# SchusterLab/quantum-optimal-control

Measured on AMD Instinct MI355X. Metric: GRAPE iterations/sec (fwd+bwd+Adam) at n=32 k=4 steps=500, higher is better.
Workload: dtype f64; 1 GPU; C2 3-transmon-size unitary gate: n=32 k=4 steps=500 m=8 Taylor(T,s)=(5,3), 64 independent control seeds per GPU (aggregate over seeds), reg_coeffs={}; seeds_per_gpu=64, total_seeds=64, chunks=16, stream_groups=1, ranks_seen=1, fidelities_gathered=64, devices_distinct=1, transport=single process, transport_fallback=False

## Files before the change

quantum-optimal-control_amd/csrc/qoc_engine.hip:

```cpp
#include "../../include/qoc.h"

#include <hip/hip_runtime.h>

#include <cmath>
#include <cstdarg>
#include <cstdio>
#include <cstdlib>
#include <cstring>
#include <string>
#include <vector>

#include "qoc_common.h"
#include "qoc_kernels_finish.h"
#include "qoc_kernels_generic.h"
#include "qoc_kernels_mfma.h"
#include "qoc_kernels_st.h"
#include "qoc_kernels_gemm.h"
#include "qoc_gemm_ts.h"
#include "qoc_small.h"

#include "qoc_plan_limits.h"
static thread_local std::string g_err;

static int fail(int code, const char* fmt, ...) {
// ... 182 lines not shown
    }
    if (d.has_speed) {
        const size_t g = ((size_t)d.B * (d.steps + 1) + 3) / 4;
        hipLaunchKernelGGL(k_time_overlaps, dim3((unsigned)(g > 4096 ? 4096 : g)), dim3(256), 0, s, d);
    }
    hipLaunchKernelGGL(k_loss, dim3(d.B), dim3(QOC_BLOCK), 0, s, d);
}

static int enqueue_small(qoc_engine* e, const QocAdamDev& ap, int iters) {
    QocDev d = e->d;
    d.skip_done = ap.mode == 1 ? 1 : 0;
    std::string msg;
    TRY(prof_begin(e));
    const int rc = qoc_small_launch(e->sm, d, ap, iters, e->stream, msg);
    if (rc) return fail(rc == -1 ? QOC_ERR_INVALID : QOC_ERR_HIP, "workgroup-resident iteration: %s", msg.c_str());
    TRY(prof_end(e));
    HIP_TRY(hipGetLastError());
    e->evaluated = true;
    e->controls_ready = false;
    e->final_stale = true;
    e->inter_stale = true;
    return QOC_OK;
}

static int enqueue_iteration(qoc_engine* e, const QocAdamDev& ap) {
    if (e->path == QOC_PATH_SMALL) return enqueue_small(e, ap, 1);
    const bool own_controls = e->path == QOC_PATH_MFMA && e->mf.latency && e->mf.NT == 2;
    const bool swap_in = e->controls_ready && !own_controls && !(e->skip_mask & 1);
    if (swap_in) { std::swap(e->d.u, e->d.u2); std::swap(e->d.w, e->d.w2); }
    e->controls_ready = false;
    QocDev d = e->d;
    if (own_controls) { d.u2 = nullptr; d.w2 = nullptr; }
    d.skip_done = ap.mode == 1 ? 1 : 0;
    d.uscale_in_loss = (e->path == QOC_PATH_MFMA && !e->mf.latency && !e->mf.updown) ? 1 : 0;
    const int total = d.B * d.k * d.steps;
    int cgrid = (total + QOC_BLOCK - 1) / QOC_BLOCK;
    if (cgrid > 2048) cgrid = 2048;
    const int skip = e->skip_mask;
    const bool plain = !(d.has_amp || d.has_env || d.has_dwdt || d.has_d2wdt2 || d.has_band);
    const bool fused_tail = e->path == QOC_PATH_MFMA && e->mf.latency && (!e->mf.lat_sources || e->mf.lat_src_fast) && !d.has_band
        && !(skip & (16 | 32));
    if (!(skip & 1) && !own_controls && !swap_in) hipLaunchKernelGGL(k_controls, dim3(cgrid), dim3(QOC_BLOCK), 0, e->stream, d);
    if (e->path == QOC_PATH_MFMA) {
        TRY(prof_begin(e));
        if (!(skip & 2)) qoc_mfma_launch_expm(e->mf, d, e->stream);
        TRY(prof_end(e));
// ... 22 lines not shown
        qoc_gemm_backward(e->gm, d, e->stream);
        if (bracket_bwd) TRY(prof_end(e));
        }
    } else if (!d.state_transfer) {
        TRY(prof_begin(e));
        hipLaunchKernelGGL(k_expm_generic, dim3(e->expm_grid), dim3(QOC_BLOCK), 0, e->stream, d, e->K, e->expm_scratch);
        TRY(prof_end(e));
        hipLaunchKernelGGL(k_fwd_generic, dim3(d.B), dim3(QOC_BLOCK), 0, e->stream, d, e->K, e->seed_scratch);
        launch_loss(d, e->stream);
        hipLaunchKernelGGL(k_bwd_generic, dim3(d.B), dim3(QOC_BLOCK), 0, e->stream, d, e->K, e->seed_scratch);
    } else if (e->path == QOC_PATH_ST_FUSED) {
        TRY(prof_begin(e));
        st_fused_launch(d, e->stream, true);
        TRY(prof_end(e));
        launch_loss(d, e->stream);
        st_fused_launch(d, e->stream, false);
    } else {
        TRY(prof_begin(e));
        hipLaunchKernelGGL(k_st_fwd_generic, dim3(d.B), dim3(QOC_BLOCK), 0, e->stream, d, e->seed_scratch);
        TRY(prof_end(e));
        launch_loss(d, e->stream);
        hipLaunchKernelGGL(k_st_bwd_generic, dim3(d.B), dim3(QOC_BLOCK), 0, e->stream, d, e->seed_scratch);
    }
    if (!(skip & 32) && !fused_tail) {
        const dim3 fb(d.k * d.steps >= 2048 ? 1024 : QOC_BLOCK);
        if (d.has_band) {
            const size_t items = (size_t)d.B * d.k * d.steps, g1 = (items + 3) / 4, g2 = (items + 255) / 256;
            hipLaunchKernelGGL(k_band_spectrum, dim3((unsigned)(g1 > 8192 ? 8192 : g1)), dim3(256), 0, e->stream, d);
            hipLaunchKernelGGL(k_band_gradient, dim3((unsigned)(g2 > 8192 ? 8192 : g2)), dim3(256), 0, e->stream, d);
        }
        const bool wide = d.k * d.steps > 4 * 1024 && d.k * d.steps <= 8 * 1024;
        const bool split = d.k * d.steps > 4 * 1024 && e->fin_part;
        if (split) {
            const dim3 sg((unsigned)e->fin_S, (unsigned)d.B);
            QocGradPartial gp{nullptr, 0, 0, 0};
            if (e->path == QOC_PATH_GEMM && e->gm.reduce_in_tail) gp = QocGradPartial{e->gm.partial, e->gm.N / 32, e->gm.ldW, e->gm.MV};
            if (plain) {
                hipLaunchKernelGGL(k_finish_split_a<true>, sg, dim3(256), 0, e->stream, d, ap, e->fin_part, gp);
                hipLaunchKernelGGL(k_finish_split_b<true>, sg, dim3(256), 0, e->stream, d, ap, e->fin_part);
            } else {
                hipLaunchKernelGGL(k_finish_split_a<false>, sg, dim3(256), 0, e->stream, d, ap, e->fin_part, gp);
                hipLaunchKernelGGL(k_finish_split_b<false>, sg, dim3(256), 0, e->stream, d, ap, e->fin_part);
            }
        }
        else if (plain && wide) hipLaunchKernelGGL((k_finish_t<true, 8>), dim3(d.B), fb, 0, e->stream, d, ap);
        else if (plain) hipLaunchKernelGGL(k_finish_t<true>, dim3(d.B), fb, 0, e->stream, d, ap);
        else if (wide) hipLaunchKernelGGL((k_finish_t<false, 8>), dim3(d.B), fb, 0, e->stream, d, ap);
        else hipLaunchKernelGGL(k_finish_t<false>, dim3(d.B), fb, 0, e->stream, d, ap);
    }
    HIP_TRY(hipGetLastError());
    e->evaluated = true;
    e->controls_ready = ap.mode != 0 && !own_controls && !(skip & (16 | 32));
    e->final_stale = (e->path == QOC_PATH_MFMA && (e->mf.latency || e->mf.updown)) ||
                     (e->path == QOC_PATH_GEMM && e->gm.ts_G <= 0 && qoc_gemm_lazy_final(e->gm, e->d));
    e->inter_stale = (e->path == QOC_PATH_MFMA && e->final_stale && (!e->mf.lat_sources || e->mf.lat_src_fast))
// ... 161 lines not shown
        ident.assign(2 * nn, 0.0);
        for (int a = 0; a < n; ++a) ident[2 * (a * n + a)] = 1.0;
        U0 = ident.data();
    }
    if ((rc = dev_upload(e, &d.Hs, (const cplx*)Hs, (size_t)(k + 1) * nn))) return bail(rc);
    if ((rc = dev_upload(e, &d.U0, (const cplx*)U0, nn))) return bail(rc);
    if ((rc = dev_upload(e, &d.V, (const cplx*)V, nm))) return bail(rc);
    if ((rc = dev_upload(e, &d.W, (const cplx*)W, nm))) return bail(rc);
    if ((rc = dev_upload(e, &d.Psi0, (const cplx*)psi0.data(), nm))) return bail(rc);
    if (d.forbid_dressed && (rc = dev_upload(e, &d.Vs, (const cplx*)Vs, nn))) return bail(rc);
    if ((rc = dev_upload(e, &d.maxA, maxA, (size_t)k))) return bail(rc);
    if (one_minus_gauss && (rc = dev_upload(e, &d.omg, one_minus_gauss, ks))) return bail(rc);
    if (cfg->n_forbidden > 0) {
        std::vector<double> fa(cfg->n_forbidden);
        for (int f = 0; f < cfg->n_forbidden; ++f) fa[f] = forbidden_coeffs[f] * inv_steps;
        if ((rc = dev_upload(e, &d.forb_state, (const int*)forbidden_states, (size_t)cfg->n_forbidden))) return bail(rc);
        if ((rc = dev_upload(e, &d.forb_a, (const double*)fa.data(), (size_t)cfg->n_forbidden))) return bail(rc);
    }

#define ALLOC(ptr, count) if ((rc = dev_alloc(e, &(ptr), (count)))) return bail(rc)
    ALLOC(d.base, B * ks); ALLOC(d.adam_m, B * ks); ALLOC(d.adam_v, B * ks);
    ALLOC(d.adam_t, (size_t)B); ALLOC(d.iters, (size_t)B); ALLOC(d.done, (size_t)B);
    ALLOC(d.w, B * ks); ALLOC(d.u, B * ks); ALLOC(d.w2, B * ks); ALLOC(d.u2, B * ks); ALLOC(d.dLdu, B * ks); ALLOC(d.grad, B * ks);
    if (ks > 4 * 1024 && !qoc_exp_is("QOC_FINISH_SPLIT", 0)) {
        e->fin_S = (int)((ks + 255) / 256);
        if (e->fin_S > 64) e->fin_S = 64;
        ALLOC(e->fin_part, (size_t)B * (e->fin_S + 2) * 2);
    }
    ALLOC(d.inter, (size_t)B * (steps + 1) * nm);
    ALLOC(d.Xfinal, (size_t)B * nn);
    ALLOC(d.ztau, (size_t)B * (steps + 1));
    if (d.n_forb > 0) ALLOC(d.Fpop, (size_t)B * (steps + 1) * d.n_forb * m);
    if (d.forbid_dressed && d.n_forb > 0) ALLOC(d.Fd, (size_t)B * (steps + 1) * d.n_forb * m);
    ALLOC(d.zfin, (size_t)B); ALLOC(d.su_resid, (size_t)B);
    ALLOC(d.loss, (size_t)B); ALLOC(d.reg_state, (size_t)B); ALLOC(d.reg_loss, (size_t)B);
    ALLOC(d.g2, (size_t)B); ALLOC(d.uscale, (size_t)B);
    if (d.has_band) { ALLOC(d.band_ph, B * ks); ALLOC(d.band_tw, (size_t)steps); ALLOC(d.band_mag, B * ks); ALLOC(d.band_dR, B * ks); }
    ALLOC(e->step_lr, (size_t)B);
    if (hipMemset(d.base, 0, B * ks * sizeof(double)) != hipSuccess ||
        hipMemset(d.adam_m, 0, B * ks * sizeof(double)) != hipSuccess ||
        hipMemset(d.adam_v, 0, B * ks * sizeof(double)) != hipSuccess ||
        hipMemset(d.adam_t, 0, B * sizeof(int)) != hipSuccess ||
        hipMemset(d.iters, 0, B * sizeof(int)) != hipSuccess ||
        hipMemset(d.done, 0, B * sizeof(int)) != hipSuccess ||
        hipMemset(d.su_resid, 0, B * sizeof(double)) != hipSuccess ||
        hipMemset(d.uscale, 0, B * sizeof(double)) != hipSuccess ||
        hipMemset(d.Xfinal, 0, (size_t)B * nn * sizeof(cplx)) != hipSuccess)
        return bail(fail(QOC_ERR_HIP, "qoc_create: clearing the state buffers failed"));
    if (d.has_band) {
        hipLaunchKernelGGL(k_band_twiddles, dim3((steps + 255) / 256), dim3(256), 0, 0, d.band_tw, steps);
        if (hipGetLastError() != hipSuccess || hipStreamSynchronize(0) != hipSuccess)
// ... 92 lines not shown
            "result of this engine is garbage (timing experiments only)\n", e->skip_mask);
    }
#endif
    if (path == QOC_PATH_MFMA) {
        std::string msg;
        e->mf.variant = latency_auto ? 5 : cfg->variant;
        if (cfg->variant == 5 && !qoc_mfma_latency_ok(d))
            return bail(fail(QOC_ERR_INVALID, "qoc_create: the latency mode of the MFMA path (variant 5) needs n <= 32 with k <= 8 (or, "
                "with at most 4 dressed forbidden levels, n <= 64), "
                                              "a Taylor degree >= 2 (n=%d k=%d T=%d)", n, k, d.T));
        d.T = qoc_mfma_degree(d);
        rc = qoc_mfma_setup(e->mf, d, cfg->chunks, (const cplx*)Hs, e->allocs, msg);
        if (rc) return bail(fail(rc, "qoc_create: %s", msg.c_str()));
        e->chunks = e->mf.C;
    } else if (path == QOC_PATH_GEMM) {
        std::string msg;
        if (cfg->time_shards >= 1) { e->gm.ts_G = cfg->time_shards; e->gm.ts_rank = cfg->time_rank; }
        e->gm.antiherm = antiherm;
        e->gm.direct_variant = cfg->path == QOC_PATH_GEMM ? cfg->variant : 0;
        rc = qoc_gemm_setup(e->gm, d, (const cplx*)Hs, gemm_direct, e->allocs, msg);
        if (rc) return bail(fail(rc, "qoc_create: %s", msg.c_str()));
        if (!qoc_gemm_lds_opt_in()) return bail(fail(QOC_ERR_HIP, "qoc_create: cannot reserve LDS for the GEMM-path kernels"));
        e->chunks = e->gm.NC;
        e->gm.reduce_in_tail = e->gm.persistent && e->fin_part != nullptr && e->skip_mask == 0;
        if (e->gm.ts_G > 0) {
            std::string why;
            if (!qoc_gemm_ts_supported(e->gm, d, e->gm.ts_G, why))
                return bail(fail(QOC_ERR_INVALID, "qoc_create: time_shards = %d needs %s (n=%d m=%d chunks=%d)", e->gm.ts_G, why.c_str(), n,
                    m, e->gm.NC));
            qoc_gemm_ts_ranges(e->gm, e->gm.ts_G);
        }
    } else if (path == QOC_PATH_SMALL) {
        std::string msg;
        rc = qoc_small_setup(e->sm, d, antiherm, cfg->chunks, cfg->variant, e->allocs, msg);
        if (rc) return bail(fail(rc == -1 ? QOC_ERR_INVALID : (rc == -3 ? QOC_ERR_NOMEM : QOC_ERR_HIP), "qoc_create: %s (n=%d m=%d k=%d T=%d steps=%d seeds=%d)",
            msg.c_str(), n, m, k, d.T, steps, B));
        e->chunks = e->sm.G;
        if (!cfg->state_transfer) {
            ALLOC(e->K, (size_t)B * steps * nn);
            int grid = B * steps;
            if (grid > 4096) grid = 4096;
            e->expm_grid = grid;
            ALLOC(e->expm_scratch, (size_t)grid * 3 * nn);
            ALLOC(e->seed_scratch, (size_t)B * (2 * nn + 2 * nm));
        } else {
            ALLOC(e->seed_scratch, (size_t)B * (nn + 3 * nm));
        }
// ... 227 lines not shown
    HIP_TRY(hipStreamSynchronize(e->stream));
    HIP_TRY(hipEventRecord(e->t0, e->stream));
    TRY(qoc_iterate(e, p, iters));
    HIP_TRY(hipEventRecord(e->t1, e->stream));
    HIP_TRY(hipEventSynchronize(e->t1));
    float ms = 0.f;
    HIP_TRY(hipEventElapsedTime(&ms, e->t0, e->t1));
    if (elapsed_ms) *elapsed_ms = ms;
    return QOC_OK;
}

int qoc_path_in_use(qoc_handle e) { return e ? e->path : QOC_ERR_INVALID; }
int qoc_chunks_in_use(qoc_handle e) { return e ? e->chunks : QOC_ERR_INVALID; }

int qoc_plan_describe(qoc_handle e, char* buf, int32_t len) {
    if (!e || !buf || len < 1) return fail(QOC_ERR_INVALID, "qoc_plan_describe: null handle or buffer");
    char tmp[256];
    if (e->path == QOC_PATH_MFMA) {
        const QocMfma& mf = e->mf;
        const bool split = (mf.NT > 2 || (mf.NT == 2 && e->d.k >= 6)) && mf.variant != 1;
        const char* sweeps = mf.latency ? (mf.lat_sources ? "latency_sources" : "latency")
                             : mf.updown ? "downup" : (split ? (mf.grad_rt ? "row_tile_gradient" : "split") : (mf.variant == 1
                                 || mf.NT == 1 || mf.NT == 4 ? "one_wave" : "pair"));
        snprintf(tmp, sizeof tmp, "path=mfma nt=%d expm=%d chunks=%d sweeps=%s", mf.NT, qoc_mfma_expm_variant(mf, e->d), mf.C, sweeps);
    } else if (e->path == QOC_PATH_GEMM) {
        const QocGemm& g = e->gm;
        int w = snprintf(tmp, sizeof tmp, "path=gemm route=%s chunks=%d slices_per_chunk=%d chains=%s",
            g.direct ? "direct" : (e->d.state_transfer ? "propagator" : "unitary"),
                         g.NC, g.S, g.persistent ? "persistent" : "launches");
        if (g.ts_G > 0) w += snprintf(tmp + w, sizeof tmp - w, " time_shards=%d time_rank=%d", g.ts_G, g.ts_rank);
        if (g.direct) snprintf(tmp + w, sizeof tmp - w, " taylor_chain=%s",
            g.sq_chain ? "squared" : g.dpp_packed ? "packed"
            : g.dpp_chain ? (g.dpp_cw == 10 ? "columns40" : g.dpp_cw == 12 ? "columns48" : g.dpp_cw == 14 ? "columns56" : "full")
                : "butterfly");
    } else if (e->path == QOC_PATH_SMALL) {
        snprintf(tmp, sizeof tmp, "path=small n_pad=%d rows=%d slices_per_row=%d workgroups=%d state_sources=%d lds_kb=%d", e->sm.N, e->sm.R, e->sm.L, e->sm.G,
            e->sm.src ? 1 : 0, (int)((e->sm.lds_bytes + 1023) / 1024));
    } else {
        snprintf(tmp, sizeof tmp, "path=%s", e->path == QOC_PATH_ST_FUSED ? "st_fused" : "generic");
    }
    snprintf(buf, (size_t)len, "%s", tmp);
    return QOC_OK;
}

}

#include "qoc_comm.h"
```

quantum-optimal-control_amd/csrc/qoc_mfma_backward.hip:

```cpp
#include "qoc_kernels_mfma.h"
#include "qoc_plan_limits.h"
#include "qoc_mfma_backward.h"
#include "qoc_mfma_downup.h"

static const void* qoc_downup_kernel(const QocDev& d) {
    const int qa = qoc_active_strips(d.n);
#define QOC_DU(KCv) (qa == 8 ? (const void*)k_mfma_downup<2, KCv, 8> : qa == 7 ? (const void*)k_mfma_downup<2, KCv, 7> : \
                     qa == 6 ? (const void*)k_mfma_downup<2, KCv, 6> : (const void*)k_mfma_downup<2, KCv, 5>)
    return d.k == 5 ? QOC_DU(5) : QOC_DU(4);
#undef QOC_DU
}

static const void* qoc_backward3_kernel(const QocMfma& mf, const QocDev& d) {
    const bool src = d.n_forb > 0 || d.has_speed;
    const int qa = qoc_active_strips(d.n);
#define QOC_B3S(MQv, KCv) (qa == 8 ? (const void*)k_mfma_backward3<MQv, true, KCv, 0, 8> : qa == 7 ? (const void*)k_mfma_backward3<MQv, true, KCv, 0, 7> : \
                           qa == 6 ? (const void*)k_mfma_backward3<MQv, true, KCv, 0, 6> : (const void*)k_mfma_backward3<MQv, true, KCv, 0, 5>)
#define QOC_B3K(MQv, KCv) (src ? QOC_B3S(MQv, KCv) : (const void*)k_mfma_backward3<MQv, false, KCv>)
    if (d.k == 5) return mf.mq <= 2 ? QOC_B3K(2, 5) : QOC_B3K(4, 5);
    return mf.mq <= 2 ? QOC_B3K(2, 4) : QOC_B3K(4, 4);
#undef QOC_B3K
#undef QOC_B3S
}

int qoc_mfma_setup(QocMfma& mf, const QocDev& d, int chunks_req, const cplx* Hs_host,
                                 std::vector<void*>& allocs, std::string& msg) {
    const int NT = (mf.variant == 5 && d.n <= 32) ? 2 : d.n <= 16 ? 1 : (d.n <= 32 ? 2 : ((d.n <= 48 && !(mf.variant == 5 && d.k > 4)) ? 3 : 4));
    const int FR = 256 * NT * NT;
    mf.NT = NT; mf.FR = FR;
    mf.updown = NT == 2 && mf.variant != 1 && mf.variant != 5 && d.k <= 5 && d.m <= 8 && !(d.n_forb > 0 || d.has_speed) &&
                !qoc_exp_is("QOC_UPDOWN", 0);
    mf.exp_rows_qa_full = qoc_exp_env("QOC_ROWS_QA_FULL") && !qoc_exp_is("QOC_ROWS_QA_FULL", 0);
    mf.exp_lat_qa8 = qoc_exp_env("QOC_LAT_QA8") && !qoc_exp_is("QOC_LAT_QA8", 0);
    mf.exp_lat_offsets_own = qoc_exp_is("QOC_LAT_OFFSETS_IN_SWEEP", 0);
    int C = chunks_req;
    if (C <= 0) {
        C = NT == 2 ? QOC_PLAN_CHUNK_ITEMS / d.Bplan : (QOC_PLAN_CHUNK_ITEMS + d.Bplan - 1) / d.Bplan;
        if (C > (NT == 2 ? QOC_PLAN_CHUNKS_MAX_NT2 : QOC_PLAN_CHUNKS_MAX)) C = NT == 2 ? QOC_PLAN_CHUNKS_MAX_NT2 : QOC_PLAN_CHUNKS_MAX;
    }
    mf.latency = mf.variant == 5;
    if (mf.latency && chunks_req <= 0) C = (d.steps + 7) / 8;
    if (C > d.steps) C = d.steps;
    if (C > (mf.latency ? 16 * QOC_MAXC : QOC_MAXC)) C = mf.latency ? 16 * QOC_MAXC : QOC_MAXC;
    if (C < 1) C = 1;
    int L = (d.steps + C - 1) / C;
    C = (d.steps + L - 1) / L;
    mf.C = C; mf.L = L;
    mf.G = 0; mf.NG = 0;
    mf.lat_sources = mf.latency && (d.n_forb > 0 || d.has_speed);
    if (mf.latency) {
        int G = 8;
        while (G * G < C) ++G;
        mf.G = G; mf.NG = (C + G - 1) / G;
    }
// ... 28 lines not shown
        std::vector<cplx> hs(hd);
        for (auto& v : hs) { v.x *= sc; v.y *= sc; }
        if (!up(&mf.HsD, hs)) { msg = "MFMA path: constant upload failed"; return -3; }
    }
    std::vector<std::pair<cplx**, size_t>> wanted;
    auto al = [&](cplx** dst, size_t count) -> bool { wanted.emplace_back(dst, (count * sizeof(cplx) + 4095) & ~(size_t)4095); return true; };
    mf.skew_c = 5 * 16;
    mf.skew_b = 3 * 16;
    const size_t nk = (size_t)d.B * ((size_t)d.steps * FR + (size_t)C * mf.skew_c + mf.skew_b), np = (size_t)d.B * C * FR;
    mf.store_T = !((NT == 2 || NT == 3) && mf.variant != 1) || mf.latency;
    const bool split_grad = (NT > 2 || (NT == 2 && d.k >= 6)) && mf.variant != 1;
    if (split_grad && !al(&mf.LamD, (size_t)d.B * d.steps * 16 * NT * 16)) { msg = "MFMA path: out of device memory"; return -3; }
    { const int kg = NT >= 4 ? 2 : 4; mf.grad_lds = (size_t)(d.k < kg ? d.k : kg) * FR * sizeof(cplx); }
    mf.grad_rt = NT >= 2 && split_grad && d.k <= 8 && !qoc_exp_is("QOC_GRAD_RT", 0);
    if (mf.grad_rt) {
        mf.grad_lds = (size_t)((d.k + 3) & ~3) * NT * 256 * sizeof(cplx);
        if (!al((cplx**)&mf.gpart, ((size_t)NT * d.B * d.k * d.steps + 1) / 2)) { msg = "MFMA path: out of device memory"; return -3; }
    }
    if (mf.updown && !al(&mf.LamL, (size_t)d.B * d.steps * NT * (mf.mq <= 2 ? 2 : 4) * 64)) { msg = "MFMA path: out of device memory"; return -3; }
    if (mf.lat_sources && !al(&mf.Goff, (size_t)d.B * mf.NG * 4 * NT * 64)) { msg = "MFMA path: out of device memory"; return -3; }
    const bool bnd = (NT == 2 || NT == 3) && mf.variant != 1 && !mf.latency;
    const bool bnd_adj = bnd && NT == 2 && d.k <= 5 && !(d.n_forb > 0 || d.has_speed);
    mf.updown = mf.updown && bnd_adj;
    const size_t nbnd = (size_t)d.B * C * NT * (mf.mq <= 2 ? 2 : 4) * 64;
    if ((bnd && !al(&mf.BndF, nbnd)) || (bnd_adj && !al(&mf.BndA, nbnd))) { msg = "MFMA path: out of device memory"; return -3; }
    const bool dressed = d.n_forb > 0 && d.forbid_dressed;
    mf.lat_src_fast = mf.lat_sources && !(dressed && d.n_forb > 4);
    mf.lat_dressed = mf.lat_src_fast && dressed;
    if (mf.lat_src_fast) {
        const size_t vec = (size_t)NT * (mf.mq <= 2 ? 2 : 4) * 64;
        if (!al(&mf.AoffL, (size_t)d.B * C * vec) || !al(&mf.GoffL, (size_t)d.B * mf.NG * vec) || !al(&mf.LamS, (size_t)d.B * d.steps * vec) ||
            !al((cplx**)&mf.loss_part, (size_t)d.B * (d.steps + 1))) { msg = "MFMA path: out of device memory"; return -3; }
    }
    if (mf.latency && (!al(&mf.GfD, (size_t)d.B * mf.NG * FR) || !al(&mf.GfT, (size_t)d.B * mf.NG * FR) || !al(&mf.TfD, (size_t)d.B * FR) ||
                       !al(&mf.PsiL, (size_t)d.B * d.steps * NT * (mf.mq <= 2 ? 2 : 4) * 64) ||
                       !al(&mf.LamL, (size_t)d.B * d.steps * NT * (mf.mq <= 2 ? 2 : 4) * 64))) { msg = "MFMA path: out of device memory"; return -3; }
    if (!al(&mf.KfD, nk) || (mf.store_T && !al(&mf.KfT, nk)) || !al(&mf.PfD, np) || !al(&mf.PfT, np) || !al(&mf.Aoff, (size_t)d.B * C * 4 * NT * 64)) { msg = "MFMA path: out of device memory"; return -3; }
    {
        size_t total = 0;
        for (auto& w : wanted) total += w.second;
        char* arena = nullptr;
        if (hipMalloc((void**)&arena, qoc_arena_bytes(total)) != hipSuccess) { msg = "MFMA path: out of device memory"; return -3; }
        allocs.push_back(arena);
        size_t off = 0;
        for (auto& w : wanted) { *w.first = (cplx*)(arena + off); off += w.second; }
        const size_t xl = (size_t)d.B * d.steps * NT * (mf.mq <= 2 ? 2 : 4) * 64 * sizeof(cplx);
// ... 14 lines not shown
    if (mf.latency) {
        if (qoc_mfma_latency_setup(mf, d, msg) != 0) return -2;
        void* p = nullptr;
        if (hipMalloc(&p, (size_t)d.B * sizeof(unsigned)) != hipSuccess) { msg = "MFMA path: out of device memory"; return -3; }
        allocs.push_back(p);
        if (hipMemset(p, 0, (size_t)d.B * sizeof(unsigned)) != hipSuccess) { msg = "MFMA path: clearing the arrival counters failed"; return -2; }
        mf.lat_count = (unsigned*)p;
    }
    if (NT == 2 && mf.lat_sources && d.k <= 5) {
#define QOC_B3L(MQv, KCv, MODEv) (const void*)k_mfma_backward3<MQv, true, KCv, MODEv>
        const void* k1 = d.k == 5 ? (mf.mq <= 2 ? QOC_B3L(2, 5, 1) : QOC_B3L(4, 5, 1)) : (mf.mq <= 2 ? QOC_B3L(2, 4, 1) : QOC_B3L(4, 4, 1));
        const void* k2 = d.k == 5 ? (mf.mq <= 2 ? QOC_B3L(2, 5, 2) : QOC_B3L(4, 5, 2)) : (mf.mq <= 2 ? QOC_B3L(2, 4, 2) : QOC_B3L(4, 4, 2));
#undef QOC_B3L
        if (hipFuncSetAttribute(k1, hipFuncAttributeMaxDynamicSharedMemorySize, (int)mf.bwd_lds3) != hipSuccess ||
            hipFuncSetAttribute(k2, hipFuncAttributeMaxDynamicSharedMemorySize, (int)mf.bwd_lds3) != hipSuccess) {
            msg = "MFMA path: cannot reserve LDS for the two-level backward kernel";
            return -2;
        }
    }
    if (NT == 2 && mf.updown) {
        const int kc = d.k == 5 ? 5 : 4, mqv = mf.mq <= 2 ? 2 : 4;
        mf.du_lds = (size_t)kc * FR * sizeof(cplx) + (size_t)8 * 4 * mqv * F2_LDP * sizeof(cplx) + (size_t)4 * 2 * NT * mqv * 64 * sizeof(cplx) +
                    (size_t)8 * 4 * kc * sizeof(double) + 8 * sizeof(int);
        if (hipFuncSetAttribute(qoc_downup_kernel(d), hipFuncAttributeMaxDynamicSharedMemorySize, (int)mf.du_lds) != hipSuccess) {
            msg = "MFMA path: cannot reserve LDS for the fused sweep kernel";
            return -2;
        }
    }
    if (NT == 2 && bnd_adj) {
        const void* k3 = d.k == 5 ? (mf.mq <= 2 ? (const void*)k_mfma_backward3<2, false, 5, 3> : (const void*)k_mfma_backward3<4, false, 5, 3>)
                                  : (mf.mq <= 2 ? (const void*)k_mfma_backward3<2, false, 4, 3> : (const void*)k_mfma_backward3<4, false, 4, 3>);
        if (hipFuncSetAttribute(k3, hipFuncAttributeMaxDynamicSharedMemorySize, (int)mf.bwd_lds3) != hipSuccess) {
            msg = "MFMA path: cannot reserve LDS for the backward kernel with precomputed boundaries";
            return -2;
        }
    }
    if (NT == 2 && hipFuncSetAttribute(b3k, hipFuncAttributeMaxDynamicSharedMemorySize, (int)mf.bwd_lds3) != hipSuccess) {
        msg = "MFMA path: cannot reserve LDS for the prefetching backward kernel";
        return -2;
    }
    if (split_grad) {
        const void* gk = NT == 2 ? (mf.mq <= 2 ? (const void*)k_mfma_grad<2, 2> : (const void*)k_mfma_grad<2, 4>)
                       : NT == 3 ? (mf.mq <= 2 ? (const void*)k_mfma_grad<3, 2> : (const void*)k_mfma_grad<3, 4>)
                                 : (mf.mq <= 2 ? (const void*)k_mfma_grad<4, 2> : (const void*)k_mfma_grad<4, 4>);
        if (mf.grad_rt)
            gk = NT == 2 ? (mf.mq <= 2 ? (const void*)k_mfma_grad_rt<2, 2> : (const void*)k_mfma_grad_rt<2, 4>)
               : NT == 3 ? (mf.mq <= 2 ? (const void*)k_mfma_grad_rt<3, 2> : (const void*)k_mfma_grad_rt<3, 4>)
// ... 24 lines not shown
            QOC_QA_SWITCH(qoc_active_strips(d.n), QOC_O2);
#undef QOC_O2
        } else {
            hipLaunchKernelGGL(k_mfma_bwd_offsets<NT>, dim3((items + 3) / 4), dim3(256), 0, s, d, mf);
        }
    }
    if (NT == 2 && mf.variant != 1) {
        if (d.k <= 5) {
            const bool src = d.n_forb > 0 || d.has_speed;
            if (mf.lat_sources) {
                const dim3 gg(d.B * mf.NG), gc(items), b1(128);
#define QOC_B3L(MQv, MODEv, GRID) do { if (d.k == 5) hipLaunchKernelGGL((k_mfma_backward3<MQv, true, 5, MODEv>), GRID, b1, mf.bwd_lds3, s, d, mf); \
                                       else hipLaunchKernelGGL((k_mfma_backward3<MQv, true, 4, MODEv>), GRID, b1, mf.bwd_lds3, s, d, mf); } while (0)
                if (mf.mq <= 2) { QOC_B3L(2, 2, gg); QOC_B3L(2, 1, gc); } else { QOC_B3L(4, 2, gg); QOC_B3L(4, 1, gc); }
#undef QOC_B3L
                return;
            }
            const dim3 g3((items + 3) / 4), b3(512);
#define QOC_B3B(MQv) do { if (d.k == 5) hipLaunchKernelGGL((k_mfma_backward3<MQv, false, 5, 3>), g3, b3, mf.bwd_lds3, s, d, mf); \
                          else hipLaunchKernelGGL((k_mfma_backward3<MQv, false, 4, 3>), g3, b3, mf.bwd_lds3, s, d, mf); } while (0)
            if (mf.updown && !src) {
                const dim3 gd((items + 3) / 4), bd(512);
                void* kargs[] = {(void*)&d, (void*)&mf};
                (void)hipLaunchKernel(qoc_downup_kernel(d), gd, bd, kargs, mf.du_lds, s);
            }
            else if (mf.BndA && !src) { if (mf.mq <= 2) QOC_B3B(2); else QOC_B3B(4); }
            else {
                void* kargs[] = {(void*)&d, (void*)&mf};
                (void)hipLaunchKernel(qoc_backward3_kernel(mf, d), g3, b3, kargs, mf.bwd_lds3, s);
            }
#undef QOC_B3B
            return;
        }
        {
#define QOC_O2F(QAv) do { if (mf.mq <= 2) hipLaunchKernelGGL((k_mfma_bwd_offsets2<2, true, QAv>), dim3((items + 3) / 4), dim3(256), 0, s, d, mf); \
                          else hipLaunchKernelGGL((k_mfma_bwd_offsets2<4, true, QAv>), dim3((items + 3) / 4), dim3(256), 0, s, d, mf); } while (0)
            QOC_QA_SWITCH(qoc_active_strips(d.n), QOC_O2F);
#undef QOC_O2F
            const int slices = d.B * d.steps;
            int gg = (slices + 3) / 4; if (gg > 2048) gg = 2048;
            if (mf.grad_rt) {
                if (gg > 512) gg = 512;
                if (mf.mq <= 2) hipLaunchKernelGGL((k_mfma_grad_rt<2, 2>), dim3(2 * gg), dim3(256), mf.grad_lds, s, d, mf);
                else hipLaunchKernelGGL((k_mfma_grad_rt<2, 4>), dim3(2 * gg), dim3(256), mf.grad_lds, s, d, mf);
                hipLaunchKernelGGL(k_mfma_grad_sum, dim3(256), dim3(256), 0, s, d, mf, 2);
            }
            else if (mf.mq <= 2) hipLaunchKernelGGL((k_mfma_grad<2, 2>), dim3(gg), dim3(256), mf.grad_lds, s, d, mf);
// ... 33 lines not shown
```

quantum-optimal-control_amd/csrc/qoc_mfma_downup.h:

```cpp
#pragma once
#include "qoc_mfma_frag.h"

template <int MQ, int KC, int QA = 8>
__global__ void __launch_bounds__(512) k_mfma_downup(QocDev d, QocMfma mf) {
    constexpr int NT = 2, LDP = F2_LDP, ISZ = 4 * MQ * LDP, VSZ = NT * MQ * 64;
    extern __shared__ __attribute__((aligned(16))) char smem[];
    const int lane = threadIdx.x & 63;
    const int wv = __builtin_amdgcn_readfirstlane(threadIdx.x >> 6);
    const int role = wv & 1, pr = wv >> 1;
    cplx* Hl = (cplx*)smem;
    cplx* img = Hl + (size_t)KC * QFR + (size_t)wv * ISZ;
    cplx* xch = Hl + (size_t)KC * QFR + (size_t)8 * ISZ + (size_t)pr * 2 * VSZ;
    double* gred = (double*)(Hl + (size_t)KC * QFR + (size_t)8 * ISZ + (size_t)4 * 2 * VSZ) + wv * 4 * KC;
    volatile int* flag = (volatile int*)((double*)(Hl + (size_t)KC * QFR + (size_t)8 * ISZ + (size_t)4 * 2 * VSZ) + 8 * 4 * KC) + pr * 2;
    for (int o = threadIdx.x; o < KC * QFR; o += blockDim.x) Hl[o] = o < d.k * QFR ? mf.HfD[QFR + o] : cmake(0.0, 0.0);
    if (lane == 0) flag[role] = 0;
    __syncthreads();
    const int item = blockIdx.x * 4 + pr;
#ifndef QOC_DOWNUP_STAGGER
#define QOC_DOWNUP_STAGGER 2
#endif
    constexpr int STG = QOC_DOWNUP_STAGGER == 4 ? 1 : (QOC_DOWNUP_STAGGER == 2 ? 2 : 0);
    if (item >= d.B * mf.C) { if (STG && lane == 0) flag[role] = 1; return; }
    const int c = item / d.B, b = item - c * d.B;
    if (d.skip_done && d.done[b]) { if (STG && lane == 0) flag[role] = 1; return; }
    if (STG && pr >= STG) {
        volatile int* prev = flag - 2 * STG;
// ... 76 lines not shown
        for (int I = 0; I < NT; ++I)
#pragma unroll
            for (int Jp = 0; Jp < NT; ++Jp) {
                d4 t1v = {0, 0, 0, 0}, t2v = {0, 0, 0, 0}, t3v = {0, 0, 0, 0};
#pragma unroll
                for (int q = 0; q < MQ; ++q) {
                    t1v = QMFMA(lr(I, q), pr_(Jp, q), t1v);
                    t2v = QMFMA(li(I, q), pi_(Jp, q), t2v);
                    t3v = QMFMA(lr(I, q) - li(I, q), pr_(Jp, q) + pi_(Jp, q), t3v);
                }
                const d4 qr = t1v + t2v, qi = t3v - t1v + t2v;
#pragma unroll
                for (int kk = 0; kk < KC; ++kk) {
                    double acc = 0.0;
#pragma unroll
                    for (int r = 0; r < 4 && 4 * I + r < QA; ++r) {
                        const cplx hv = Hl[(size_t)kk * QFR + (Jp * QQS + 4 * I + r) * 64 + lane];
                        acc = fma(hv.x, qr[r], acc);
                        acc = fma(-hv.y, qi[r], acc);
                    }
                    g[kk] += acc;
                }
            }
#pragma unroll
        for (int kk = 0; kk < KC; ++kk) {
            g[kk] += dpp_xor<1>(g[kk]); g[kk] += dpp_xor<2>(g[kk]); g[kk] += dpp_xor<4>(g[kk]); g[kk] += dpp_xor<8>(g[kk]);
        }
        if (lc == 0) {
#pragma unroll
            for (int kk = 0; kk < KC; ++kk) gred[lk * KC + kk] = g[kk];
        }
        wave_lds_fence();
        if (lane < d.k) d.dLdu[((size_t)b * d.k + lane) * d.steps + t] = (gred[lane] + gred[KC + lane]) + (gred[2 * KC + lane] + gred[3 * KC + lane]);
        asm volatile("" ::: "memory");
    };
    auto publish = [&](int which, const double (&re)[NT][MQ], const double (&im)[NT][MQ]) {
#pragma unroll
        for (int I = 0; I < NT; ++I)
#pragma unroll
            for (int jb = 0; jb < MQ; ++jb) xch[which * VSZ + (I * MQ + jb) * 64 + lane] = cmake(re[I][jb], im[I][jb]);
        wave_lds_fence();
        if (lane == 0) flag[which] = 1;
    };
    auto receive = [&](int which, double (&re)[NT][MQ], double (&im)[NT][MQ]) {
        while (flag[which] == 0) __builtin_amdgcn_s_sleep(4);
        asm volatile("" ::: "memory");
#pragma unroll
        for (int I = 0; I < NT; ++I)
#pragma unroll
            for (int jb = 0; jb < MQ; ++jb) { const cplx v = xch[which * VSZ + (I * MQ + jb) * 64 + lane]; re[I][jb] = v.x; im[I][jb] = v.y; }
        wave_lds_fence();
    };
    const size_t vec0 = ((size_t)b * mf.C + c) * VSZ + lane;
// ... 105 lines not shown
```

quantum-optimal-control_amd/csrc/qoc_mfma_frag.h:

```cpp
#pragma once
#include <string>
#include <vector>
#include "qoc_common.h"

#define QOC_NP 32
#define QOC_MAXC 64
#define QNP (16 * NT)
#define QQS (4 * NT)
#define QLDR (16 * NT + 1)
#define QFR (256 * NT * NT)
#define F2_LDP 33
static inline int qoc_active_strips(int n) { return n > 28 ? 8 : (n > 24 ? 7 : (n > 20 ? 6 : 5)); }
#define QOC_QA_SWITCH(qa, F) do { switch (qa) { case 5: F(5); break; case 6: F(6); break; case 7: F(7); break; default: F(8); break; } } while (0)
static inline int qoc_active_strips_lat(int n) { return n > 16 ? qoc_active_strips(n) : (n > 8 ? 4 : 2); }
#define QOC_QA_SWITCH_LAT(qa, F) do { switch (qa) { case 2: F(2); break; case 4: F(4); break; case 5: F(5); break; case 6: F(6); break; case 7: F(7); break; default: F(8); break; } } while (0)

typedef double d4 __attribute__((ext_vector_type(4)));
#define QMFMA(a, b, c) __builtin_amdgcn_mfma_f64_16x16x4f64((a), (b), (c), 0, 0, 0)

struct CTile { d4 re, im; };
template <int NT> struct AFragT { double re[NT][4 * NT], im[NT][4 * NT]; };

struct QocMfma {
    int C = 1;
    int L = 1;
    int mq = 4;
    int NT = 2;
    int FR = 1024;
    double invfact[24];
    double pcoef[24];
    double psigma = 1.0;
    cplx* HsD = nullptr;
    cplx* HfD = nullptr;
    cplx* HfT = nullptr;
    cplx* U0fD = nullptr;
    cplx* KfD = nullptr;
    cplx* KfT = nullptr;
    bool store_T = true;
    cplx* PfD = nullptr;
    cplx* PfT = nullptr;
    cplx* BndF = nullptr;
    cplx* BndA = nullptr;
    bool updown = false;
    size_t du_lds = 0;
    cplx* Aoff = nullptr;
    cplx* Goff = nullptr;
    cplx* LamD = nullptr;
    size_t grad_lds = 0;
    double* gpart = nullptr;
    int grad_rt = 0;
    size_t bwd_lds = 0, bwd_lds3 = 0;
    bool h_in_lds = true;
    int variant = 0;
    int G = 0, NG = 0;
    cplx* GfD = nullptr;
    cplx* TfD = nullptr;
    cplx* PsiL = nullptr;
    cplx* LamL = nullptr;
    cplx* LamS = nullptr;
    cplx* AoffL = nullptr;
    cplx* GoffL = nullptr;
    bool lat_dressed = false;
    bool exp_rows_qa_full = false, exp_lat_qa8 = false, exp_lat_offsets_own = false;
    bool lat_src_fast = false;
    double* loss_part = nullptr;
    unsigned* lat_count = nullptr;
// ... 187 lines not shown
```

quantum-optimal-control_amd/csrc/qoc_plan_limits.h:

```cpp
#pragma once

#define QOC_PLAN_LAT_WORK 4608
#define QOC_PLAN_LAT_WORK_SRC 4096
#define QOC_PLAN_LAT_WORK_PER_STRIP 512
#define QOC_PLAN_LAT_WORK_PER_STRIP_SRC 768
#define QOC_PLAN_LAT_WORK_NT3 16384
#define QOC_PLAN_LAT_WORK_NT4 4096
#define QOC_PLAN_LAT_SETS_N16 6
#define QOC_PLAN_LAT_SETS_N16_ST 8
#define QOC_PLAN_LAT_SETS_N32 16
#define QOC_PLAN_LAT_SETS_N32_ST_WIDE 4
#define QOC_PLAN_LAT_SETS_NT3 8
#define QOC_PLAN_LAT_SETS_NT4 4
#define QOC_PLAN_LAT_MIN_SLICES 64
#define QOC_PLAN_LAT_SINGLE_MAX_SLICES 8192
#define QOC_PLAN_NT3_MIN_SETS 8
#define QOC_PLAN_NT4_MIN_SETS_K4 32
#define QOC_PLAN_NT4_MIN_SETS 64
#define QOC_PLAN_GEMM_SMALL_MIN_SLICES 100
#define QOC_PLAN_GEMM_SMALL_Q5 2
#define QOC_PLAN_GEMM_SMALL_Q6 3
#define QOC_PLAN_GEMM_SMALL_Q7 5
#define QOC_PLAN_GEMM_SMALL_Q8 7
#define QOC_PLAN_GEMM_SMALL_SRC_Q5 5
#define QOC_PLAN_GEMM_SMALL_SRC_Q6 6
#define QOC_PLAN_GEMM_SMALL_SRC_Q78 8
#define QOC_PLAN_GEMM_SMALL_ST_WIDE 8
#define QOC_PLAN_ST_BIG_N32 112
#define QOC_PLAN_ST_BIG_N32_MIN_LEVELS 20
#define QOC_PLAN_ST_BIG_N32_MIN_LEVELS_SRC 28
#define QOC_PLAN_ST_BIG_N64 48
#define QOC_PLAN_ST_BIG_N64_SRC 112
#define QOC_PLAN_ST_BIG_DPP 20
#define QOC_PLAN_ST_BIG_DPP_SRC 48
#define QOC_PLAN_ST_DIRECT_N32 112
#define QOC_PLAN_ST_DIRECT_N64 48
#define QOC_PLAN_ST_DIRECT_DPP 12
#define QOC_PLAN_ST_DIRECT_DPP_SRC 22
#define QOC_PLAN_CHUNK_ITEMS 1024
#define QOC_PLAN_CHUNKS_MAX_NT2 64
#define QOC_PLAN_CHUNKS_MAX 32
#define QOC_PLAN_SMALL_MAX_MODEL_US 52
#define QOC_PLAN_SMALL_MODEL_US_BASE 36
#define QOC_PLAN_SMALL_MODEL_NS_PER_SLICE 36
#define QOC_PLAN_SMALL_MAX_MODEL_US_SRC 85
#define QOC_PLAN_SMALL_MAX_SETS 256
```

Measured before the change: 60250 GRAPE iterations/s.

## Split finish tail for mid-size few-seed runs and add butterfly sweep gradient reduction

Result: no change. 60830 GRAPE iterations/s, median of 6 (+1.0%).

```diff
diff --git a/quantum-optimal-control_amd/csrc/qoc_engine.hip b/quantum-optimal-control_amd/csrc/qoc_engine.hip
--- a/quantum-optimal-control_amd/csrc/qoc_engine.hip
+++ b/quantum-optimal-control_amd/csrc/qoc_engine.hip
@@ -228,6 +228,13 @@
     e->inter_stale = true;
     return QOC_OK;
 }
+
+static int finish_split_S(long long ks, int B) {
+    if (qoc_exp_is("QOC_FINISH_SPLIT", 0)) return 0;
+    if (ks <= QOC_PLAN_TAIL_SPLIT_ELEMS && !(ks >= QOC_PLAN_TAIL_SPLIT_MIN_ELEMS && B <= QOC_PLAN_TAIL_SPLIT_MAX_SETS)) return 0;
+    return (int)std::min<long long>((ks + 255) / 256, 64);
+}
+static bool uses_split_tail(const qoc_engine* e) { return e->fin_part != nullptr; }
 
 static int enqueue_iteration(qoc_engine* e, const QocAdamDev& ap) {
     if (e->path == QOC_PATH_SMALL) return enqueue_small(e, ap, 1);
@@ -296,6 +303,8 @@
         launch_loss(d, e->stream);
         hipLaunchKernelGGL(k_st_bwd_generic, dim3(d.B), dim3(QOC_BLOCK), 0, e->stream, d, e->seed_scratch);
     }
+    if (e->path == QOC_PATH_GEMM && e->gm.reduce_in_tail && (fused_tail || (skip & 32) || !uses_split_tail(e)))
+        return fail(QOC_ERR_STATE, "enqueue_iteration: the gradient partials are left to a split tail that does not run");
     if (!(skip & 32) && !fused_tail) {
         const dim3 fb(d.k * d.steps >= 2048 ? 1024 : QOC_BLOCK);
         if (d.has_band) {
@@ -304,7 +313,7 @@
             hipLaunchKernelGGL(k_band_gradient, dim3((unsigned)(g2 > 8192 ? 8192 : g2)), dim3(256), 0, e->stream, d);
         }
         const bool wide = d.k * d.steps > 4 * 1024 && d.k * d.steps <= 8 * 1024;
-        const bool split = d.k * d.steps > 4 * 1024 && e->fin_part;
+        const bool split = uses_split_tail(e);
         if (split) {
             const dim3 sg((unsigned)e->fin_S, (unsigned)d.B);
             QocGradPartial gp{nullptr, 0, 0, 0};
@@ -512,11 +521,7 @@
     ALLOC(d.base, B * ks); ALLOC(d.adam_m, B * ks); ALLOC(d.adam_v, B * ks);
     ALLOC(d.adam_t, (size_t)B); ALLOC(d.iters, (size_t)B); ALLOC(d.done, (size_t)B);
     ALLOC(d.w, B * ks); ALLOC(d.u, B * ks); ALLOC(d.w2, B * ks); ALLOC(d.u2, B * ks); ALLOC(d.dLdu, B * ks); ALLOC(d.grad, B * ks);
-    if (ks > 4 * 1024 && !qoc_exp_is("QOC_FINISH_SPLIT", 0)) {
-        e->fin_S = (int)((ks + 255) / 256);
-        if (e->fin_S > 64) e->fin_S = 64;
-        ALLOC(e->fin_part, (size_t)B * (e->fin_S + 2) * 2);
-    }
+    if ((e->fin_S = finish_split_S((long long)ks, (int)B)) > 0) ALLOC(e->fin_part, (size_t)B * (e->fin_S + 2) * 2);
     ALLOC(d.inter, (size_t)B * (steps + 1) * nm);
     ALLOC(d.Xfinal, (size_t)B * nn);
     ALLOC(d.ztau, (size_t)B * (steps + 1));
@@ -655,7 +660,7 @@
         if (rc) return bail(fail(rc, "qoc_create: %s", msg.c_str()));
         if (!qoc_gemm_lds_opt_in()) return bail(fail(QOC_ERR_HIP, "qoc_create: cannot reserve LDS for the GEMM-path kernels"));
         e->chunks = e->gm.NC;
-        e->gm.reduce_in_tail = e->gm.persistent && e->fin_part != nullptr && e->skip_mask == 0;
+        e->gm.reduce_in_tail = e->gm.persistent && uses_split_tail(e) && e->skip_mask == 0;
         if (e->gm.ts_G > 0) {
             std::string why;
             if (!qoc_gemm_ts_supported(e->gm, d, e->gm.ts_G, why))
@@ -929,7 +934,8 @@
         const char* sweeps = mf.latency ? (mf.lat_sources ? "latency_sources" : "latency")
                              : mf.updown ? "downup" : (split ? (mf.grad_rt ? "row_tile_gradient" : "split") : (mf.variant == 1
                                  || mf.NT == 1 || mf.NT == 4 ? "one_wave" : "pair"));
-        snprintf(tmp, sizeof tmp, "path=mfma nt=%d expm=%d chunks=%d sweeps=%s", mf.NT, qoc_mfma_expm_variant(mf, e->d), mf.C, sweeps);
+        const int w = snprintf(tmp, sizeof tmp, "path=mfma nt=%d expm=%d chunks=%d sweeps=%s", mf.NT, qoc_mfma_expm_variant(mf, e->d), mf.C, sweeps);
+        if (mf.updown && !mf.latency) snprintf(tmp + w, sizeof tmp - w, " sweep_reduce=%s", mf.du_bfly ? "butterfly" : "per_value");
     } else if (e->path == QOC_PATH_GEMM) {
         const QocGemm& g = e->gm;
         int w = snprintf(tmp, sizeof tmp, "path=gemm route=%s chunks=%d slices_per_chunk=%d chains=%s",
@@ -946,6 +952,11 @@
     } else {
         snprintf(tmp, sizeof tmp, "path=%s", e->path == QOC_PATH_ST_FUSED ? "st_fused" : "generic");
     }
+    if (e->path != QOC_PATH_SMALL && !(e->path == QOC_PATH_MFMA && e->mf.latency)) {
+        const size_t w = strlen(tmp);
+        if (uses_split_tail(e)) snprintf(tmp + w, sizeof tmp - w, " tail=split tail_workgroups=%d", e->fin_S);
+        else snprintf(tmp + w, sizeof tmp - w, " tail=single");
+    }
     snprintf(buf, (size_t)len, "%s", tmp);
     return QOC_OK;
 }
diff --git a/quantum-optimal-control_amd/csrc/qoc_mfma_backward.hip b/quantum-optimal-control_amd/csrc/qoc_mfma_backward.hip
--- a/quantum-optimal-control_amd/csrc/qoc_mfma_backward.hip
+++ b/quantum-optimal-control_amd/csrc/qoc_mfma_backward.hip
@@ -3,11 +3,11 @@
 #include "qoc_mfma_backward.h"
 #include "qoc_mfma_downup.h"
 
-static const void* qoc_downup_kernel(const QocDev& d) {
+static const void* qoc_downup_kernel(const QocMfma& mf, const QocDev& d) {
     const int qa = qoc_active_strips(d.n);
-#define QOC_DU(KCv) (qa == 8 ? (const void*)k_mfma_downup<2, KCv, 8> : qa == 7 ? (const void*)k_mfma_downup<2, KCv, 7> : \
-                     qa == 6 ? (const void*)k_mfma_downup<2, KCv, 6> : (const void*)k_mfma_downup<2, KCv, 5>)
-    return d.k == 5 ? QOC_DU(5) : QOC_DU(4);
+#define QOC_DU(KCv, BFv) (qa == 8 ? (const void*)k_mfma_downup<2, KCv, 8, BFv> : qa == 7 ? (const void*)k_mfma_downup<2, KCv, 7, BFv> : \
+                          qa == 6 ? (const void*)k_mfma_downup<2, KCv, 6, BFv> : (const void*)k_mfma_downup<2, KCv, 5, BFv>)
+    return d.k == 5 ? QOC_DU(5, false) : (mf.du_bfly ? QOC_DU(4, true) : QOC_DU(4, false));
 #undef QOC_DU
 }
 
@@ -30,6 +30,7 @@
     mf.NT = NT; mf.FR = FR;
     mf.updown = NT == 2 && mf.variant != 1 && mf.variant != 5 && d.k <= 5 && d.m <= 8 && !(d.n_forb > 0 || d.has_speed) &&
                 !qoc_exp_is("QOC_UPDOWN", 0);
+    mf.du_bfly = mf.updown && d.k <= 4 && !qoc_exp_is("QOC_UPDOWN_BUTTERFLY", 0);
     mf.exp_rows_qa_full = qoc_exp_env("QOC_ROWS_QA_FULL") && !qoc_exp_is("QOC_ROWS_QA_FULL", 0);
     mf.exp_lat_qa8 = qoc_exp_env("QOC_LAT_QA8") && !qoc_exp_is("QOC_LAT_QA8", 0);
     mf.exp_lat_offsets_own = qoc_exp_is("QOC_LAT_OFFSETS_IN_SWEEP", 0);
@@ -104,6 +105,7 @@
     const bool bnd = (NT == 2 || NT == 3) && mf.variant != 1 && !mf.latency;
     const bool bnd_adj = bnd && NT == 2 && d.k <= 5 && !(d.n_forb > 0 || d.has_speed);
     mf.updown = mf.updown && bnd_adj;
+    mf.du_bfly = mf.du_bfly && mf.updown;
     const size_t nbnd = (size_t)d.B * C * NT * (mf.mq <= 2 ? 2 : 4) * 64;
     if ((bnd && !al(&mf.BndF, nbnd)) || (bnd_adj && !al(&mf.BndA, nbnd))) { msg = "MFMA path: out of device memory"; return -3; }
     const bool dressed = d.n_forb > 0 && d.forbid_dressed;
@@ -164,7 +166,7 @@
         const int kc = d.k == 5 ? 5 : 4, mqv = mf.mq <= 2 ? 2 : 4;
         mf.du_lds = (size_t)kc * FR * sizeof(cplx) + (size_t)8 * 4 * mqv * F2_LDP * sizeof(cplx) + (size_t)4 * 2 * NT * mqv * 64 * sizeof(cplx) +
                     (size_t)8 * 4 * kc * sizeof(double) + 8 * sizeof(int);
-        if (hipFuncSetAttribute(qoc_downup_kernel(d), hipFuncAttributeMaxDynamicSharedMemorySize, (int)mf.du_lds) != hipSuccess) {
+        if (hipFuncSetAttribute(qoc_downup_kernel(mf, d), hipFuncAttributeMaxDynamicSharedMemorySize, (int)mf.du_lds) != hipSuccess) {
             msg = "MFMA path: cannot reserve LDS for the fused sweep kernel";
             return -2;
         }
@@ -235,7 +237,7 @@
             if (mf.updown && !src) {
                 const dim3 gd((items + 3) / 4), bd(512);
                 void* kargs[] = {(void*)&d, (void*)&mf};
-                (void)hipLaunchKernel(qoc_downup_kernel(d), gd, bd, kargs, mf.du_lds, s);
+                (void)hipLaunchKernel(qoc_downup_kernel(mf, d), gd, bd, kargs, mf.du_lds, s);
             }
             else if (mf.BndA && !src) { if (mf.mq <= 2) QOC_B3B(2); else QOC_B3B(4); }
             else {
diff --git a/quantum-optimal-control_amd/csrc/qoc_mfma_downup.h b/quantum-optimal-control_amd/csrc/qoc_mfma_downup.h
--- a/quantum-optimal-control_amd/csrc/qoc_mfma_downup.h
+++ b/quantum-optimal-control_amd/csrc/qoc_mfma_downup.h
@@ -1,8 +1,9 @@
 #pragma once
 #include "qoc_mfma_frag.h"
 
-template <int MQ, int KC, int QA = 8>
+template <int MQ, int KC, int QA = 8, bool BF = false>
 __global__ void __launch_bounds__(512) k_mfma_downup(QocDev d, QocMfma mf) {
+    static_assert(!BF || KC == 4, "k_mfma_downup: the butterfly reduction needs four control images");
     constexpr int NT = 2, LDP = F2_LDP, ISZ = 4 * MQ * LDP, VSZ = NT * MQ * 64;
     extern __shared__ __attribute__((aligned(16))) char smem[];
     const int lane = threadIdx.x & 63;
@@ -125,6 +126,15 @@
                     g[kk] += acc;
                 }
             }
+        if constexpr (BF) {
+            const bool b0 = lane & 1, b1 = lane & 2;
+            double w[2];
+#pragma unroll
+            for (int p = 0; p < 2; ++p) w[p] = (b0 ? g[2 * p + 1] : g[2 * p]) + dpp_xor<1>(b0 ? g[2 * p] : g[2 * p + 1]);
+            double y = (b1 ? w[1] : w[0]) + dpp_xor<2>(b1 ? w[0] : w[1]);
+            y += dpp_xor<4>(y); y += dpp_xor<8>(y);
+            if (lc < 4) gred[lk * KC + lc] = y;
+        } else {
 #pragma unroll
         for (int kk = 0; kk < KC; ++kk) {
             g[kk] += dpp_xor<1>(g[kk]); g[kk] += dpp_xor<2>(g[kk]); g[kk] += dpp_xor<4>(g[kk]); g[kk] += dpp_xor<8>(g[kk]);
@@ -132,6 +142,7 @@
         if (lc == 0) {
 #pragma unroll
             for (int kk = 0; kk < KC; ++kk) gred[lk * KC + kk] = g[kk];
+        }
         }
         wave_lds_fence();
         if (lane < d.k) d.dLdu[((size_t)b * d.k + lane) * d.steps + t] = (gred[lane] + gred[KC + lane]) + (gred[2 * KC + lane] + gred[3 * KC + lane]);
diff --git a/quantum-optimal-control_amd/csrc/qoc_mfma_frag.h b/quantum-optimal-control_amd/csrc/qoc_mfma_frag.h
--- a/quantum-optimal-control_amd/csrc/qoc_mfma_frag.h
+++ b/quantum-optimal-control_amd/csrc/qoc_mfma_frag.h
@@ -42,6 +42,7 @@
     cplx* BndF = nullptr;
     cplx* BndA = nullptr;
     bool updown = false;
+    bool du_bfly = false;
     size_t du_lds = 0;
     cplx* Aoff = nullptr;
     cplx* Goff = nullptr;
diff --git a/quantum-optimal-control_amd/csrc/qoc_plan_limits.h b/quantum-optimal-control_amd/csrc/qoc_plan_limits.h
--- a/quantum-optimal-control_amd/csrc/qoc_plan_limits.h
+++ b/quantum-optimal-control_amd/csrc/qoc_plan_limits.h
@@ -40,6 +40,9 @@
 #define QOC_PLAN_CHUNK_ITEMS 1024
 #define QOC_PLAN_CHUNKS_MAX_NT2 64
 #define QOC_PLAN_CHUNKS_MAX 32
+#define QOC_PLAN_TAIL_SPLIT_ELEMS 4096
+#define QOC_PLAN_TAIL_SPLIT_MIN_ELEMS 1024
+#define QOC_PLAN_TAIL_SPLIT_MAX_SETS 64
 #define QOC_PLAN_SMALL_MAX_MODEL_US 52
 #define QOC_PLAN_SMALL_MODEL_US_BASE 36
 #define QOC_PLAN_SMALL_MODEL_NS_PER_SLICE 36
```
